# imatge-upc/rsis

Measured on AMD Instinct MI355X. Metric: training images/sec at 256x256, T=10, batch=32 per GPU, higher is better.
Workload: dtype f32

## Files before the change

include/rsis_hip.h:

```cpp
#ifndef RSIS_HIP_H
#define RSIS_HIP_H
#include <stddef.h>
#ifdef __cplusplus
extern "C" {
#endif

#define RSIS_ABI_VERSION 2

#define RSIS_DTYPE_F32 0
#define RSIS_DTYPE_BF16 1
#define RSIS_DTYPE_BF16_BLK 2
#define RSIS_DTYPE_F32_WINO 3

int rsis_version(void);
const char* rsis_error_string(int code);
int rsis_conv_uses_wino(int ks, int stride, int pad, int Cin, int Cout, int nseg, int lstm_hid);

int rsis_set_deterministic(int on);
int rsis_get_deterministic(void);

int rsis_conv_uses_bf16(int ks, int stride, int pad, int Cout);
long rsis_conv_packed_bytes_fwd(int dtype, int Cout, int ks, int stride, int pad, int nseg, const int* Cseg);
long rsis_conv_packed_bytes_dgrad(int dtype, int Cout, int ks, int stride, int pad, int c_count);
int rsis_conv_pack_fwd(const float* W, void* Wp, int Cout, int Ctot, int ks, int stride, int pad, int nseg, const int* Cseg,
// ... 52 lines not shown
typedef struct rsis_lstm_bwd_job {
  const float* dh;
  const float* dh2;
  const float* dc_next;
  const float* act;
  const float* c_prev;
  const float* c;
  float* da;
  float* dc_prev;
  int B, hid, HW;
} rsis_lstm_bwd_job;
int rsis_convlstm_bwd_gates_batch(const rsis_lstm_bwd_job* jobs, int njobs, void* stream);
typedef struct rsis_dgrad_job {
  const float* dy;
  int B, Cout, Hy, Wy;
  const void* Wd;
  int Cin_packed, ks, stride, pad;
  float* dx[3];
  int Cdx[3];
  int ndst, Hx, Wx;
  const float* addend;
  int tile, dtype;
} rsis_dgrad_job;
int rsis_conv2d_dgrad_batch(const rsis_dgrad_job* jobs, int njobs, void* stream);

int rsis_upsample_bilinear_ac_fwd(const float* x, float* y, long BC, int Hi, int Wi, int Ho, int Wo, void* stream);
int rsis_upsample_bilinear_ac_bwd(const float* dy, float* dx, long BC, int Hi, int Wi, int Ho, int Wo, void* stream);
int rsis_upsample_maxpool_bwd(const float* dy, const float* dpool, const int* argmax, float* dx, long BC, int Hi, int Wi, int Ho,
                              int Wo, void* stream);

int rsis_global_maxpool_fwd(const float* x, float* y, int* argmax, long BC, int HW, void* stream);
int rsis_global_maxpool_bwd(const float* dy, const int* argmax, float* dx, long BC, int HW, void* stream);
int rsis_global_maxpool_bwd_add(const float* dy, const int* argmax, float* dx, long BC, int HW, void* stream);

int rsis_bn_fwd(const float* x, const float* res, float* y, double* stats, const float* gamma, const float* beta,
                float* running_mean, float* running_var, float* save_mean, float* save_rstd, int B, int C, int HW,
                float eps, float momentum, int relu, int train, void* stream);
int rsis_bn_bwd(const float* dy, const float* x, const float* y, const float* save_mean, const float* save_rstd,
                const float* gamma, double* stats, float* dx, float* dres, float* dgamma, float* dbeta, int B, int C,
                int HW, int relu, void* stream);

int rsis_bn_bwd_eval(const float* dy, const float* x, const float* y, const float* running_mean, const float* running_var,
                     const float* gamma, double* stats, float* dx, float* dres, float* dgamma, float* dbeta, int B, int C, int HW,
                     float eps, int relu, void* stream);

int rsis_bn_fwd_mask(const float* x, const float* res, float* y, unsigned char* mask, double* stats, const float* gamma, const float* beta,
// ... 206 lines not shown
```

rsis_amd/_lib.py:

```python
import ctypes
import os

import torch

_HERE = os.path.dirname(os.path.abspath(__file__))
LIB_PATH = os.environ.get("RSIS_HIP_LIB") or os.path.join(_HERE, "lib", "librsis_hip.so")

_vp, _i, _l, _f = ctypes.c_void_p, ctypes.c_int, ctypes.c_long, ctypes.c_float
_ip = ctypes.POINTER(ctypes.c_int)
_vpp = ctypes.POINTER(ctypes.c_void_p)

class PackJob(ctypes.Structure):
    _fields_ = [("W", ctypes.c_void_p), ("out", ctypes.c_void_p), ("dgrad", ctypes.c_int), ("dtype", ctypes.c_int), ("Cout", ctypes.c_int),
                ("Ctot", ctypes.c_int), ("ks", ctypes.c_int), ("stride", ctypes.c_int), ("pad", ctypes.c_int),
                ("nseg", ctypes.c_int), ("Cseg", ctypes.c_int * 3), ("Coff", ctypes.c_int * 3), ("lstm_hid", ctypes.c_int),
                ("imode", ctypes.c_int), ("ldw", ctypes.c_int), ("krows", ctypes.c_int), ("block_begin", ctypes.c_int)]


class WgradJob(ctypes.Structure):
    _fields_ = [("dy", ctypes.c_void_p), ("x", ctypes.c_void_p), ("dW", ctypes.c_void_p)] + \
               [(k, ctypes.c_int) for k in ("B", "Cs", "H", "W", "Cout", "Ho", "Wo", "ks", "stride", "pad", "Ctot", "c_off", "lstm_hid", "dtype")]


class LstmJob(ctypes.Structure):
# ... 30 lines not shown


class BlkLstmBwdJob(ctypes.Structure):
    _fields_ = [(k, ctypes.c_void_p) for k in ("dh", "dh2", "dc_next", "act", "c_prev", "c", "da", "dc_prev")] + \
               [(k, ctypes.c_int) for k in ("B", "hid", "HW")]


SIGNATURES = {
    "rsis_version": (_i, []),
    "rsis_error_string": (ctypes.c_char_p, [_i]),
    "rsis_set_deterministic": (_i, [_i]),
    "rsis_get_deterministic": (_i, []),
    "rsis_conv_uses_bf16": (_i, [_i, _i, _i, _i]),
    "rsis_conv_uses_wino": (_i, [_i, _i, _i, _i, _i, _i, _i]),
    "rsis_conv_packed_bytes_fwd": (_l, [_i, _i, _i, _i, _i, _i, _ip]),
    "rsis_conv_packed_bytes_dgrad": (_l, [_i, _i, _i, _i, _i, _i]),
    "rsis_conv_pack_fwd": (_i, [_vp, _vp, _i, _i, _i, _i, _i, _i, _ip, _ip, _i, _i, _vp]),
    "rsis_conv_pack_dgrad": (_i, [_vp, _vp, _i, _i, _i, _i, _i, _i, _ip, _ip, _i, _i, _vp]),
    "rsis_conv_pack_job_fill": (_i, [ctypes.POINTER(PackJob)]),
    "rsis_conv_pack_batch": (_i, [_vp, _i, _i, _vp]),
    "rsis_conv2d_fwd": (_i, [_vpp, _ip, _i, _i, _i, _i, _vp, _i, _i, _i, _i, _vp, _vp, _vp, _i, _i, _i, _i, _vp]),
    "rsis_conv2d_fwd_bn_eval": (_i, [_vpp, _ip, _i, _i, _i, _i, _vp, _i, _i, _i, _i, _vp, _vp, _vp, _vp, _vp, _vp, _f, _i, _vp, _i, _i, _i, _i, _vp]),
    "rsis_conv2d_dgrad": (_i, [_vp, _i, _i, _i, _i, _vp, _i, _i, _i, _i, _vpp, _ip, _i, _i, _i, _vp, _i, _i, _vp]),
    "rsis_conv2d_wgrad": (_i, [_vp, _vp, _vp, _i, _i, _i, _i, _i, _i, _i, _i, _i, _i, _i, _i, _i, _i, _vp]),
    "rsis_conv2d_wgrad_batch": (_i, [ctypes.POINTER(WgradJob), _i, _vp]),
    "rsis_affine_nearest": (_i, [_vp, _vp, _vp, _i, _i, _i, _i, _i, _vp]),
    "rsis_targets_work_ints": (_l, [_i]),
    "rsis_targets_from_maps": (_i, [_vp, _vp, _i, _i, _i, _i, _vp, _vp, _vp, _vp, _vp, _vp]),
    "rsis_instance_maps_work_ints": (_l, [_i]),
    "rsis_instance_maps": (_i, [_vp, _vp, _i, _i, _i, _i, _vp, _vp, _vp, _vp]),
    "rsis_palette_to_ids": (_i, [_vp, _l, _vp, _i, _vp, _vp]),
    "rsis_idmap_rle_encode": (_i, [_vp, _i, _i, _vp, _i, _vp, _i, _vp, _vp]),
    "rsis_conv_out_wgrad": (_i, [_vp, _vp, _vp, _vp, _i, _i, _i, _i, _vp]),
    "rsis_conv_out_seq_fwd": (_i, [_vp, _vp, _vp, _vp, _i, _i, _i, _i, _i, _vp]),
    "rsis_conv_out_seq_dgrad": (_i, [_vp, _vp, _vp, _i, _i, _i, _i, _i, _vp]),
    "rsis_conv_out_seq_wgrad": (_i, [_vp, _vp, _vp, _vp, _i, _i, _i, _i, _i, _vp]),
    "rsis_sum_leading": (_i, [_vp, _vp, _i, _l, _vp]),
    "rsis_bias_grad": (_i, [_vp, _vp, _i, _i, _i, _i, _vp]),
    "rsis_convlstm_fwd": (_i, [_vpp, _ip, _i, _i, _i, _i, _vp, _vp, _vp, _vp, _vp, _vp, _vp, _i, _i, _i, _i, _i, _vp]),
    "rsis_convlstm_fwd_batch": (_i, [ctypes.POINTER(LstmJob), _i, _vp]),
    "rsis_convlstm_bwd_gates": (_i, [_vp, _vp, _vp, _vp, _vp, _vp, _vp, _vp, _vp, _i, _i, _i, _vp]),
    "rsis_upsample_bilinear_ac_fwd": (_i, [_vp, _vp, _l, _i, _i, _i, _i, _vp]),
    "rsis_upsample_bilinear_ac_bwd": (_i, [_vp, _vp, _l, _i, _i, _i, _i, _vp]),
    "rsis_upsample_maxpool_bwd": (_i, [_vp, _vp, _vp, _vp, _l, _i, _i, _i, _i, _vp]),
    "rsis_global_maxpool_fwd": (_i, [_vp, _vp, _vp, _l, _i, _vp]),
    "rsis_global_maxpool_bwd": (_i, [_vp, _vp, _vp, _l, _i, _vp]),
# ... 129 lines not shown
```

rsis_amd/csrc/api.hip:

```cpp
#include "common.h"
#include "../../include/rsis_hip.h"
#include <stdlib.h>

int rsis_launch_conv_igemm(ConvArgs& a, int ks, bool dgrad, int epi, int force_tile, hipStream_t st);
int rsis_launch_conv_wgrad(WgradArgs& a, int ks, hipStream_t st);
int rsis_launch_conv3x3_direct(ConvArgs& a, int epi, int force_variant, hipStream_t st);
int rsis_launch_conv_wino(const float* x, const void* U, const float* bias, const float* addend, float* y, int B, int C, int Cout, int H, int W,
                          hipStream_t st, int precise);
int rsis_launch_conv_wino_group(int n, const float* const* x, const void* const* U, float* const* y, float* const* y1, const int* B, const int* C,
                                const int* Cout, const int* C0, const int* H, const int* W, hipStream_t st);
int rsis_launch_convlstm_direct_group(ConvArgs* jobs, int n, const int* force_variant, hipStream_t st);
int rsis_launch_conv3x3_direct_group_plain(ConvArgs* jobs, int n, const int* force_variant, hipStream_t st);
int rsis_l_lstm_bwd_group(const void* const*, const int*, int, hipStream_t);
int rsis_launch_conv_bf16(ConvArgs& a, int ks, int epi, int force_variant, hipStream_t st);
int rsis_launch_conv_blk(ConvArgs& a, int ks, int variant, hipStream_t st);
int rsis_l_blk_from_nchw(const float*, void*, int, int, int, hipStream_t);
int rsis_l_blk_to_nchw(const void*, float*, int, int, int, hipStream_t);
long rsis_l_blk_bn_scratch(int);
int rsis_l_blk_bn_fwd(const void*, const void*, void*, double*, const float*, const float*, float*, float*, float*, float*, int, int, int, float,
                      float, int, int, hipStream_t);
int rsis_l_blk_bn_bwd(const void*, const void*, const void*, double*, const float*, const float*, const float*, const float*, void*, void*,
                      float*, float*, int, int, int, int, int, hipStream_t);
int rsis_l_blk_subsample(const void*, void*, long, int, int, int, int, int, hipStream_t);
int rsis_l_blk_upscatter(const void*, void*, long, int, int, int, int, int, hipStream_t);
// ... 394 lines not shown
  }
  if (use_direct_f2(ks, stride, pad))
    return rsis_launch_conv3x3_direct(a, 3, direct_variant(tile), (hipStream_t)stream);
  return rsis_launch_conv_igemm(a, ks, false, 0, tile, (hipStream_t)stream);
}

int rsis_conv2d_fwd(const float* const* src, const int* Csrc, int nsrc, int B, int H, int W, const void* Wp, int Cout,
                    int ks, int stride, int pad, const float* bias, const float* addend, float* out, int Ho, int Wo,
                    int tile, int dtype, void* stream) {
  return conv2d_fwd_impl(src, Csrc, nsrc, B, H, W, Wp, Cout, ks, stride, pad, bias, addend, out, Ho, Wo, tile, dtype, stream, nullptr);
}

int rsis_conv2d_fwd_bn_eval(const float* const* src, const int* Csrc, int nsrc, int B, int H, int W, const void* Wp, int Cout,
                            int ks, int stride, int pad, const float* bias, const float* addend, const float* gamma, const float* beta,
                            const float* running_mean, const float* running_var, float eps, int relu, float* out, int Ho, int Wo,
                            int tile, int dtype, void* stream) {
  const BnEval bn = {gamma, beta, running_mean, running_var, eps, relu};
  return conv2d_fwd_impl(src, Csrc, nsrc, B, H, W, Wp, Cout, ks, stride, pad, bias, addend, out, Ho, Wo, tile % 100, dtype, stream, &bn);
}

int rsis_conv2d_dgrad(const float* dy, int B, int Cout, int Hy, int Wy, const void* Wd, int Cin_packed, int ks, int stride,
                      int pad, float* const* dx, const int* Cdx, int ndst, int Hx, int Wx, const float* addend, int tile,
                      int dtype, void* stream) {
  if (!dy || !Wd || !dx || !Cdx || ndst < 1 || ndst > RSIS_MAX_SRC) return RSIS_ERR_ARG;
  const bool inplace = addend && ndst == 1 && stride > 1 && ks == 1 && pad == 0 && addend == dx[0];
  if (addend && !inplace && (ndst != 1 || stride != 1)) return RSIS_ERR_UNSUPPORTED;
  if (stride != 1 && stride != 2 && stride != 4) return RSIS_ERR_UNSUPPORTED;
  ConvArgs a = {};
  const float* srcs[1] = {dy};
  const int cs[1] = {Cout};
  int rc = fill_sources(a, srcs, cs, 1, ks);
  if (rc) return rc;
  int ctot = 0;
  for (int i = 0; i < ndst; ++i) { if (!dx[i] || Cdx[i] < 1) return RSIS_ERR_ARG; a.dst[i] = dx[i]; a.Cd[i] = Cdx[i]; ctot += Cdx[i]; }
  a.ndst = ndst;
  a.B = B; a.H = Hy; a.W = Wy; a.Ho = Hx; a.Wo = Wx; a.stride = stride; a.pad = pad; a.sshift = log2i(stride);
  if (ctot > Cin_packed) return RSIS_ERR_ARG;
  a.ostride = 1; a.oH = Hx; a.oW = Wx; a.ksplit = 1;
  a.wp = (const float*)Wd; a.ldw = rsis_roundup(Cin_packed, RSIS_LDW_ALIGN); a.Cout = ctot; a.bias = nullptr; a.addend = addend;
  if (dtype == RSIS_DTYPE_F32_WINO && wino_geom_dgrad(ks, stride, pad, Cin_packed, Cout)) {
    if (ndst > 2 || ctot % 32 != 0 || Cdx[0] % 32 != 0 || Hx != Hy || Wx != Wy || (ndst == 2 && addend)) return RSIS_ERR_UNSUPPORTED;
    if (ndst == 1) return rsis_launch_conv_wino(dy, Wd, nullptr, addend, dx[0], B, Cout, ctot, Hy, Wy, (hipStream_t)stream, 0);
    const float* xs[1] = {dy}; const void* us[1] = {Wd}; float* y0[1] = {dx[0]}; float* y1[1] = {dx[1]};
    const int b1[1] = {B}, c1[1] = {Cout}, co1[1] = {ctot}, c01[1] = {Cdx[0]}, h1[1] = {Hy}, w1[1] = {Wy};
    return rsis_launch_conv_wino_group(1, xs, us, y0, y1, b1, c1, co1, c01, h1, w1, (hipStream_t)stream);
  }
  if (use_bf16(dtype, ks, stride, pad, Cout)) {
// ... 24 lines not shown
      return rsis_l_c1_dgrad(dy, (const float*)Wd, a.ldw, dx[0], B, Cdx[0], Hx, Wx, 1, (hipStream_t)stream);
    {
      const bool splitk_ok = conv_splitk_ok();
      const int nq = (Cout + RSIS_CK - 1) / RSIS_CK;
      const long px_tiles = (long)B * rsis_cdiv(Hx, 8) * rsis_cdiv(Wx, Wx <= 8 ? 8 : 16);
      if (splitk_ok && !addend && nq >= 32 && px_tiles * rsis_cdiv(ctot, 64) < 160) {
        for (int i = 0; i < ndst; ++i)
          if (rsis_zero_async(dx[i], sizeof(float) * (size_t)B * Cdx[i] * Hx * Wx, (hipStream_t)stream) != RSIS_OK) return RSIS_ERR_LAUNCH;
        a.ksplit = 0;
      }
    }
    return rsis_launch_conv3x3_direct(a, 0, direct_variant(tile), (hipStream_t)stream);
  }
  if (use_direct_s2(ks, stride, pad) && ndst == 1 && Cdx[0] == Cin_packed && Hy == (Hx + 1) / 2 && Wy == (Wx + 1) / 2) {
    a.Ho = Hy; a.Wo = Wy; a.oH = Hx; a.oW = Wx;
    return rsis_launch_conv3x3_direct(a, 2, direct_variant(tile), (hipStream_t)stream);
  }
  if (ks == 1 && pad == 0 && stride > 1) {
    for (int i = 0; i < ndst && !inplace; ++i)
      if (rsis_zero_async(dx[i], sizeof(float) * (size_t)B * Cdx[i] * Hx * Wx, (hipStream_t)stream) != RSIS_OK) return RSIS_ERR_LAUNCH;
    a.Ho = Hy; a.Wo = Wy; a.stride = 1; a.sshift = 0; a.ostride = stride;
    return rsis_launch_conv_igemm(a, ks, false, 0, tile, (hipStream_t)stream);
  }
  return rsis_launch_conv_igemm(a, ks, true, 0, tile, (hipStream_t)stream);
}

static int wgrad_route(WgradArgs& a, int ks, int lstm_hid, int dtype) {
  if (dtype == RSIS_DTYPE_BF16_BLK) {
    a.blk = 1;
    return rsis_wgrad_bf16_supported(a, ks) ? 1 : -1;
  }
  if (use_direct(ks, a.stride, a.pad) && a.Cout == 1 && lstm_hid == 0 && rsis_c1_supported(a.Cs) && a.H == a.Ho && a.W == a.Wo && a.W % 4 == 0)
    return 0;
  if (dtype == RSIS_DTYPE_BF16 && rsis_wgrad_bf16_supported(a, ks)) return 1;
  static const bool tiled_ok = !(getenv("RSIS_WGRAD_TILED") && getenv("RSIS_WGRAD_TILED")[0] == '0');
  if (tiled_ok && rsis_wgrad_tiled_supported(a, ks)) return 2;
  return 3;
}
static int wgrad_fill(WgradArgs& a, const float* dy, const float* x, float* dW, int B, int Cs, int H, int W, int Cout, int Ho, int Wo,
                      int ks, int stride, int pad, int Ctot, int c_off, int lstm_hid) {
  if (!dy || !x || !dW || c_off < 0 || c_off + Cs > Ctot) return RSIS_ERR_ARG;
  a = WgradArgs{};
  a.dy = dy; a.x = x; a.dw = dW; a.B = B; a.Cs = Cs; a.H = H; a.W = W; a.Ho = Ho; a.Wo = Wo; a.Cout = Cout;
  a.stride = stride; a.pad = pad; a.ldo = Ctot * ks * ks; a.n_off = c_off * ks * ks; a.interleave_hid = lstm_hid;
  return RSIS_OK;
}
// ... 639 lines not shown
```

rsis_amd/csrc/common.h:

```cpp
#pragma once
#include <hip/hip_runtime.h>
#include <stdint.h>

#define RSIS_OK 0
#define RSIS_ERR_ARG 1
#define RSIS_ERR_LAUNCH 2
#define RSIS_ERR_UNSUPPORTED 3

#define RSIS_KPAD 32
#define RSIS_CK 8
#define RSIS_CKB3 16
#define RSIS_CKB1 64
#define RSIS_LDW_ALIGN 128
#define RSIS_MAX_SRC 3

typedef float f32x16 __attribute__((ext_vector_type(16)));
typedef float f32x4 __attribute__((ext_vector_type(4)));

static inline int rsis_check_launch() {
  hipError_t e = hipGetLastError();
  return e == hipSuccess ? RSIS_OK : RSIS_ERR_LAUNCH;
}

int rsis_zero_async(void* p, size_t bytes, hipStream_t st);
// ... 40 lines not shown
  int Ho, Wo;
  int stride, pad, sshift;
  const float* wp;
  int ldw;
  int Cout;
  const float* bias;
  const float* addend;
  const float* ep_gamma; const float* ep_beta; const float* ep_mean; const float* ep_var;
  float ep_eps;
  int ep_relu, ep_round;
  float* dst[RSIS_MAX_SRC];
  int Cd[RSIS_MAX_SRC];
  int ndst;
  int n_co_tiles, n_px_tiles;
  int ostride, oH, oW;
  int ksplit;
  int hid;
  const float* c_prev;
  float* h_out;
  float* c_out;
  float* act_out;
  unsigned long long* side_key;
  int precise;
};

__device__ __forceinline__ unsigned long long rsis_side_key(float v, int idx) {
  unsigned u = __float_as_uint(v);
  u = (u & 0x80000000u) ? ~u : (u | 0x80000000u);
  return ((unsigned long long)u << 32) | (unsigned)(0x7FFFFFFF - idx);
}
__device__ __forceinline__ float rsis_side_value(unsigned long long k) {
  unsigned u = (unsigned)(k >> 32);
  u = (u & 0x80000000u) ? (u & 0x7FFFFFFFu) : ~u;
  return __uint_as_float(u);
}
__device__ __forceinline__ int rsis_side_index(unsigned long long k) { return 0x7FFFFFFF - (int)(unsigned)(k & 0xFFFFFFFFull); }
__device__ __forceinline__ unsigned long long rsis_key_max32(unsigned long long k) {
#pragma unroll
  for (int o = 16; o > 0; o >>= 1) {
    const unsigned long long t = __shfl_xor(k, o, 64);
    k = t > k ? t : k;
  }
  return k;
}

#define RSIS_SIDE_CHECK_TILES 192
// ... 87 lines not shown
```

rsis_amd/csrc/conv_igemm.hip:

```cpp
#include "common.h"
#include <type_traits>

enum { EPI_PLAIN = 0, EPI_LSTM = 1, EPI_BN = 2 };
#ifndef RSIS_GEMM_NST_DEFAULT
#define RSIS_GEMM_NST_DEFAULT 2
#endif

typedef const float __attribute__((address_space(1)))* gcf_t;
typedef const char __attribute__((address_space(1)))* gcc_t;
typedef float __attribute__((address_space(1)))* gf_t;
typedef const f32x4 __attribute__((address_space(1)))* gcf4_t;

typedef __attribute__((address_space(3))) void* lds_vp_t;
template <int BM, int BN, int BK, int WGM, int WGN, int KS, bool DGRAD, int EPI, bool V4, int NST = 2>
__global__ __launch_bounds__(256) void conv_igemm_kernel(const ConvArgs p) {
#if __HIP_DEVICE_COMPILE__
  constexpr int TM = BM / WGM / 32, TN = BN / WGN / 32;
  constexpr int KK = KS * KS;
  constexpr int B_ROWS = 256 / BN;
  constexpr int B_LOADS = BK / B_ROWS;
  constexpr int A_F4 = BK * BM / 4;
  constexpr int A_LOADS = (A_F4 + 255) / 256;
  static_assert(WGM * WGN == 4, "4 waves per block");
  static_assert(BN == 64 || BN == 128 || BN == 256, "BN");
  static_assert(RSIS_KPAD % BK == 0, "BK must divide the packed K padding");
  static_assert(!V4 || (KS == 1 && !DGRAD), "V4 is the 1x1 GEMM path");
// ... 216 lines not shown
    if constexpr (V4) {
      __builtin_amdgcn_s_waitcnt(0x0F70);
    } else {
      if (more) RSIS_STORE_TILE(cur ^ 1)
    }
    __syncthreads();
  }
  }
#undef RSIS_LOAD_TILE
#undef RSIS_STORE_TILE
#undef RSIS_DMA_TILE

  if constexpr (EPI == EPI_BN) {
    if (tid < BM) {
      const int row = co_t * BM + tid;
      float sc = 0.f, sh = 0.f;
      if (row < p.Cout) rsis_bn_affine(rsis_bn_eval_rstd(p.ep_var[row], p.ep_eps), p.ep_gamma[row], p.ep_beta[row], p.ep_mean[row], sc, sh);
      lds[tid] = sc; lds[BM + tid] = sh;
    }
    __syncthreads();
  }
  const int co_base = co_t * BM + wm * TM * 32;
  const gcf_t bias = (gcf_t)p.bias, addend = (gcf_t)p.addend;
  if (EPI == EPI_PLAIN || EPI == EPI_BN) {
    const gf_t d0 = (gf_t)p.dst[0], d1 = (gf_t)p.dst[1], d2 = (gf_t)p.dst[2];
    const int Cd0 = p.Cd[0], Cd1 = p.Cd[1], Cd2 = p.Cd[2], Cout = p.Cout;
    const int e1 = Cd0, e2 = Cd0 + Cd1;
    const int ostride = p.ostride, oHW = p.oH * p.oW;
#pragma unroll
    for (int j = 0; j < TN; ++j) {
      const int opx = px_t * BN + wn * TN * 32 + j * 32 + l31;
      if (opx >= Npx) continue;
      const int ob = opx / HoWo;
      int osp = opx - ob * HoWo;
      if (ostride > 1) { const int oho = osp / Wo; osp = (oho * ostride) * p.oW + (osp - oho * Wo) * ostride; }
      if (p.ndst == 1 && (size_t)p.B * Cout * oHW * 4 < (1ull << 31)) {
        const unsigned span = (unsigned)((size_t)p.B * Cout * oHW * 4);
        const __amdgpu_buffer_rsrc_t ro = __builtin_amdgcn_make_buffer_rsrc((void*)p.dst[0], 0, span, 0x00020000);
        const __amdgpu_buffer_rsrc_t ra = __builtin_amdgcn_make_buffer_rsrc((void*)(addend ? p.addend : p.dst[0]), 0, span, 0x00020000);
        const unsigned rowb = (unsigned)oHW * 4u;
#pragma unroll
        for (int i = 0; i < TM; ++i) {
          const int row0 = co_base + i * 32 + 4 * hi;
          const unsigned vo = (unsigned)((ob * Cout + row0) * oHW + osp) * 4u;
          const int rows_left = Cout - row0;
          float av[16];
          if (addend) {
#pragma unroll
            for (int r = 0; r < 16; ++r) {
              const int k = (r & 3) + 8 * (r >> 2);
              av[r] = __builtin_bit_cast(float, __builtin_amdgcn_raw_buffer_load_b32(ra, k < rows_left ? vo + k * rowb : 0x7FFFFFF0u, 0, 0));
            }
          }
          if constexpr (EPI == EPI_BN) {
            const float* tab = lds + wm * TM * 32 + i * 32 + 4 * hi;
#pragma unroll
            for (int g = 0; g < 4; ++g) {
              const f32x4 s4 = *reinterpret_cast<const f32x4*>(tab + 8 * g), h4 = *reinterpret_cast<const f32x4*>(tab + BM + 8 * g);
#pragma unroll
              for (int kk = 0; kk < 4; ++kk) {
                const int r = 4 * g + kk, k = kk + 8 * g;
                float v = acc[i][j][r];
                if (bias) v += k < rows_left ? bias[row0 + k] : 0.f;
                v = rsis_bn_apply(v, s4[kk], h4[kk], addend ? av[r] : 0.f, p.ep_relu);
                __builtin_amdgcn_raw_buffer_store_b32(__builtin_bit_cast(unsigned, v), ro, k < rows_left ? vo + k * rowb : 0x7FFFFFF0u, 0, 0);
              }
            }
            continue;
          }
#pragma unroll
          for (int r = 0; r < 16; ++r) {
            const int k = (r & 3) + 8 * (r >> 2);
            float v = acc[i][j][r];
            if (bias) v += k < rows_left ? bias[row0 + k] : 0.f;
            if (addend) v += av[r];
            __builtin_amdgcn_raw_buffer_store_b32(__builtin_bit_cast(unsigned, v), ro, k < rows_left ? vo + k * rowb : 0x7FFFFFF0u, 0, 0);
// ... 60 lines not shown
          const size_t sidx = ((size_t)ob * hid + jh) * HoWo + osp;
          const float cp = c_prev ? c_prev[sidx] : 0.f;
          const float c = gf * cp + gi * gg;
          const float h = go * tanhf(c);
          c_out[sidx] = c;
          h_out[sidx] = h;
          if (act_out) {
            act_out[gidx] = gi; act_out[gidx + HoWo] = gf;
            act_out[gidx + 2 * (size_t)HoWo] = go; act_out[gidx + 3 * (size_t)HoWo] = gg;
          }
        }
      }
    }
  }
#endif
}

template <int BM, int BN, int BK, int WGM, int WGN, int KS, bool DGRAD, int EPI>
static int launch_cfg(ConvArgs& a, hipStream_t st) {
  const long Npx = (long)a.B * a.Ho * a.Wo;
  a.n_co_tiles = rsis_cdiv(a.Cout, BM);
  a.n_px_tiles = rsis_cdiv(Npx, BN);
  const int grid = a.n_co_tiles * 8 * rsis_cdiv(a.n_px_tiles, 8);
  if constexpr (KS == 1 && !DGRAD && (EPI == EPI_PLAIN || EPI == EPI_BN)) {
    if (a.stride == 1 && a.pad == 0 && a.nsrc == 1 && (a.H * a.W) % 4 == 0 && a.C[0] % BK == 0 &&
        (long)a.B * a.C[0] * a.H * a.W * 4 < (1L << 31)) {
      if constexpr (BM == 64 && BN == 64 && BK == 32 && EPI == EPI_PLAIN) {
        static const int nst = getenv("RSIS_GEMM_NST") ? atoi(getenv("RSIS_GEMM_NST")) : RSIS_GEMM_NST_DEFAULT;
        if (nst == 3) { hipLaunchKernelGGL((conv_igemm_kernel<BM, BN, BK, WGM, WGN, KS, DGRAD, EPI, true, 3>), dim3(grid), dim3(256), 0, st, a); return rsis_check_launch(); }
        if (nst == 4) { hipLaunchKernelGGL((conv_igemm_kernel<BM, BN, BK, WGM, WGN, KS, DGRAD, EPI, true, 4>), dim3(grid), dim3(256), 0, st, a); return rsis_check_launch(); }
      }
      hipLaunchKernelGGL((conv_igemm_kernel<BM, BN, BK, WGM, WGN, KS, DGRAD, EPI, true>), dim3(grid), dim3(256), 0, st, a);
      return rsis_check_launch();
    }
  }
  hipLaunchKernelGGL((conv_igemm_kernel<BM, BN, BK, WGM, WGN, KS, DGRAD, EPI, false>), dim3(grid), dim3(256), 0, st, a);
  return rsis_check_launch();
}

template <int KS, bool DGRAD, int EPI>
static int launch_ks(ConvArgs& a, hipStream_t st, int force_tile) {
  const long Npx = (long)a.B * a.Ho * a.Wo;
  int tile = force_tile;
  if (tile <= 0) {
    if (a.Cout <= 32) tile = (Npx >= 256L * 256) ? 1 : 2;
    else if (KS == 1) tile = 5;
    else if (a.Cout <= 64) tile = 3;
    else {
      const long b128 = (long)rsis_cdiv(a.Cout, 128) * rsis_cdiv(Npx, 128);
      tile = (b128 >= 200) ? 4 : ((b128 >= 100) ? 6 : 5);
// ... 5 lines not shown
    case 2: return launch_cfg<32, 128, 16, 1, 4, KS, DGRAD, EPI>(a, st);
    case 3: return launch_cfg<64, 128, 16, 2, 2, KS, DGRAD, EPI>(a, st);
    case 4: return launch_cfg<128, 128, 16, 2, 2, KS, DGRAD, EPI>(a, st);
    case 5: return launch_cfg<64, 64, 16, 2, 2, KS, DGRAD, EPI>(a, st);
    case 6: return launch_cfg<128, 64, 16, 2, 2, KS, DGRAD, EPI>(a, st);
    case 11: return launch_cfg<32, 256, 32, 1, 4, KS, DGRAD, EPI>(a, st);
    case 12: return launch_cfg<32, 128, 32, 1, 4, KS, DGRAD, EPI>(a, st);
    case 13: return launch_cfg<64, 128, 32, 2, 2, KS, DGRAD, EPI>(a, st);
    case 14: return launch_cfg<128, 128, 32, 2, 2, KS, DGRAD, EPI>(a, st);
    case 15: return launch_cfg<64, 64, 32, 2, 2, KS, DGRAD, EPI>(a, st);
    case 16: return launch_cfg<128, 64, 32, 2, 2, KS, DGRAD, EPI>(a, st);
    default: return RSIS_ERR_ARG;
  }
}

int rsis_launch_conv_igemm(ConvArgs& a, int ks, bool dgrad, int epi, int force_tile, hipStream_t st) {
  if (a.nsrc < 0 || a.nsrc > RSIS_MAX_SRC) return RSIS_ERR_ARG;
  if (epi == EPI_LSTM) {
    if (dgrad) return RSIS_ERR_UNSUPPORTED;
    if (ks == 3) return launch_ks<3, false, EPI_LSTM>(a, st, force_tile);
    if (ks == 1) return launch_ks<1, false, EPI_LSTM>(a, st, force_tile);
    return RSIS_ERR_UNSUPPORTED;
  }
  if (a.ep_gamma) {
    if (dgrad || epi != EPI_PLAIN || a.ndst != 1 || a.Cout <= 32 || a.Cout % 4 != 0 || (size_t)a.B * a.Cout * a.oH * a.oW * 4 >= (1ull << 31))
      return RSIS_ERR_UNSUPPORTED;
    if (ks == 1) return launch_cfg<64, 64, 32, 2, 2, 1, false, EPI_BN>(a, st);
    if (ks == 7 && a.Cout <= 64) return launch_cfg<64, 128, 32, 2, 2, 7, false, EPI_BN>(a, st);
    return RSIS_ERR_UNSUPPORTED;
  }
  if (!dgrad) {
    if (ks == 1) return launch_ks<1, false, EPI_PLAIN>(a, st, force_tile);
    if (ks == 3) return launch_ks<3, false, EPI_PLAIN>(a, st, force_tile);
    if (ks == 7) return launch_ks<7, false, EPI_PLAIN>(a, st, force_tile);
  } else {
    if (ks == 1 && a.stride == 1 && a.pad == 0) return launch_ks<1, false, EPI_PLAIN>(a, st, force_tile);
    if (ks == 1) return launch_ks<1, true, EPI_PLAIN>(a, st, force_tile);
    if (ks == 3) return launch_ks<3, true, EPI_PLAIN>(a, st, force_tile);
    if (ks == 7) return launch_ks<7, true, EPI_PLAIN>(a, st, force_tile);
  }
  return RSIS_ERR_UNSUPPORTED;
}
```

rsis_amd/ops.py:

```python
import ctypes
import os
import weakref

import torch

from . import _lib
from ._lib import check, int_array, lib, ptr, ptr_array, require_cuda_f32, stream

_WEIGHT_EPOCH = [0]


FORCE_TILE = [0]


DIRECT_GRAD = [False]


def _direct_target(param):
    g = param.grad if DIRECT_GRAD[0] and param is not None else None
    return g if (g is not None and g.is_contiguous() and g.dtype == torch.float32 and g.is_cuda) else None


DTYPE_F32, DTYPE_BF16 = 0, 1
DTYPE_F32_WINO = 3
# ... 161 lines not shown
            L = lib()
            Cout, Ctot = w.shape[0], w.shape[1]
            nseg, segs, offs = self._seg_args()
            n = L.rsis_conv_packed_bytes_dgrad(self.dtype, Cout, self.ks, self.stride, self.pad, self.cin) // 4
            if self.wd is None or self.wd.numel() != n:
                self.wd = torch.zeros(n, dtype=torch.float32, device=w.device)
            check(L.rsis_conv_pack_dgrad(ptr(w.detach()), ptr(self.wd), Cout, Ctot, self.ks, self.stride, self.pad, nseg, segs, offs,
                                         self.lstm_hid, self.dtype, stream()), "rsis_conv_pack_dgrad")
            self._key_d = key
            if self._refs is None:
                self._refs = (weakref.ref(w), None)
            _PACKS.add(self)
        return self.wd


def _contig(t):
    return t if t.is_contiguous() else t.contiguous()


def _conv_out_size(n, ks, stride, pad):
    return (n + 2 * pad - ks) // stride + 1


def _dgrad_all(L, dy, wd, cin_packed, ks, stride, pad, srcs, Hx, Wx, addend=None, inplace=False, dtype=DTYPE_F32):
    B, Cout, Hy, Wy = dy.shape
    shapes = [tuple(s.shape) if torch.is_tensor(s) else tuple(s) for s in srcs]
    dxs = [addend] if inplace else [torch.empty(sh, dtype=torch.float32, device=dy.device) for sh in shapes]
    check(L.rsis_conv2d_dgrad(ptr(dy), B, Cout, Hy, Wy, ptr(wd), cin_packed, ks, stride, pad, ptr_array(dxs),
                              int_array([sh[1] for sh in shapes]), len(shapes), Hx, Wx, ptr(addend), FORCE_TILE[0], dtype, stream()),
          "rsis_conv2d_dgrad")
    return dxs


class GradSlot(object):

    def __init__(self):
        self.grad = None
        self.done = False

    def reset(self):
        self.grad, self.done = None, False

    def take(self):
        g, self.grad = self.grad, None
        self.done = True
        return g

    def park(self, g):
        if self.done or self.grad is not None or g is None:
            return False
        self.grad = g
        return True


class _GradTapFn(torch.autograd.Function):
    @staticmethod
    def forward(ctx, x, slot):
        ctx.slot = slot
        return x.view_as(x)

    @staticmethod
    def backward(ctx, g):
        if g is not None and ctx.slot.park(g if g.is_contiguous() else g.contiguous()):
            return None, None
        return g, None


def grad_tap(x, slot):
    if slot is None or not (torch.is_grad_enabled() and x.requires_grad):
        return x
    return _GradTapFn.apply(x, slot)


WGRAD_DEFER = [False]
_WGRAD_QUEUE = []
# ... 23 lines not shown
def _wgrad_all(L, dy, srcs, w_shape, ks, stride, pad, lstm_hid, out=None, dtype=DTYPE_F32):
    B, Cout, Ho, Wo = dy.shape
    Ctot = w_shape[1]
    dW = out if out is not None else torch.zeros(w_shape, dtype=torch.float32, device=dy.device)
    c_off = 0
    for s in srcs:
        _, Cs, H, W = s.shape
        wgrad_launch(L, dy, s, dW, B, Cs, H, W, Cout, Ho, Wo, ks, stride, pad, Ctot, c_off, lstm_hid, dtype, "rsis_conv2d_wgrad",
                     out is not None)
        c_off += Cs
    return dW


class _Conv2dFn(torch.autograd.Function):
    @staticmethod
    def forward(ctx, pack, stride, pad, nsrc, slot, *tensors):
        srcs = [_contig(t) for t in tensors[:nsrc]]
        weight, bias = tensors[nsrc], tensors[nsrc + 1]
        ctx.slot = slot
        require_cuda_f32(weight, bias, *srcs)
        L = lib()
        B, _, H, W = srcs[0].shape
        Cout, ks = weight.shape[0], weight.shape[2]
        Ho, Wo = _conv_out_size(H, ks, stride, pad), _conv_out_size(W, ks, stride, pad)
        if pack.stride != stride or pack.pad != pad:
            raise _lib.RsisHipError("PackedConv was built for stride %d pad %d, used with %d/%d" % (pack.stride, pack.pad, stride, pad))
        wp = pack.fwd(weight)
        out = torch.empty((B, Cout, Ho, Wo), dtype=torch.float32, device=weight.device)
        ctx.in_shape = None
        if ks == 1 and stride > 1 and pad == 0 and nsrc == 1 and (SUBSAMPLE_1X1[0] or pack.dtype == DTYPE_BF16):
            ctx.in_shape = tuple(srcs[0].shape)
            sub = torch.empty((B, srcs[0].shape[1], Ho, Wo), dtype=torch.float32, device=weight.device)
            check(L.rsis_subsample2d(ptr(srcs[0]), ptr(sub), B * srcs[0].shape[1], H, W, stride, stream()), "rsis_subsample2d")
            srcs = [sub]
            H, W, stride_k = Ho, Wo, 1
        else:
            stride_k = stride
        tile = FORCE_TILE[0] + (100 if pack.training_call else 0)
        check(L.rsis_conv2d_fwd(ptr_array(srcs), int_array([s.shape[1] for s in srcs]), nsrc, B, H, W, ptr(wp), Cout, ks, stride_k,
                                pad, ptr(bias.detach() if bias is not None else None), None, ptr(out), Ho, Wo, tile, pack.dtype, stream()),
              "rsis_conv2d_fwd")
        ctx.pack, ctx.stride, ctx.pad, ctx.nsrc = pack, stride, pad, nsrc
        ctx.has_bias = bias is not None
        ctx.wparam, ctx.bparam = weight, bias
        ctx.save_for_backward(weight, *srcs)
        return out

    @staticmethod
    def backward(ctx, dy):
        weight = ctx.saved_tensors[0]
        srcs = list(ctx.saved_tensors[1:])
        dy = _contig(dy)
        L = lib()
        ks = weight.shape[2]
        nsrc = ctx.nsrc
        grads = [None] * (nsrc + 2)
        take, park = ctx.slot if isinstance(ctx.slot, tuple) else (ctx.slot, None)
        addend = take.take() if take is not None else None
        sub = ctx.in_shape is not None
        in_shapes = [ctx.in_shape] if sub else [tuple(t.shape) for t in srcs]
        if any(ctx.needs_input_grad[5:5 + nsrc]):
            wd = ctx.pack.dgrad(weight)
            inplace, extra = False, None
            if addend is not None:
                if nsrc != 1 or tuple(addend.shape) != in_shapes[0]:
                    raise _lib.RsisHipError("GradSlot: the parked gradient does not belong to this conv's input")
                if ctx.stride != 1:
                    if ks == 1 and ctx.pad == 0 and addend.is_contiguous():
                        inplace = True
                    else:
                        extra, addend = addend, None
            dxs = _dgrad_all(L, dy, wd, ctx.pack.cin, ks, ctx.stride, ctx.pad, in_shapes, in_shapes[0][2], in_shapes[0][3], addend,
                             inplace, dtype=ctx.pack.dtype)
            if extra is not None:
                dxs[0].add_(extra)
            for i in range(nsrc):
                if ctx.needs_input_grad[5 + i]:
                    grads[i] = dxs[i]
            if park is not None and nsrc == 1 and grads[0] is not None and park.park(grads[0]):
                grads[0] = None
        want_w = ctx.needs_input_grad[5 + nsrc]
        want_b = ctx.has_bias and ctx.needs_input_grad[6 + nsrc]
        if (want_w and want_b and weight.shape[0] == 1 and ks == 3 and ctx.stride == 1 and ctx.pad == 1 and nsrc == 1 and
                weight.shape[1] in (4, 8, 16) and srcs[0].shape[3] % 4 == 0):
            tw, tb = _direct_target(ctx.wparam), _direct_target(ctx.bparam)
            dW = tw if tw is not None else torch.zeros_like(weight)
            db = tb if tb is not None else torch.zeros(1, dtype=torch.float32, device=dy.device)
            x0 = srcs[0]
            check(L.rsis_conv_out_wgrad(ptr(dy), ptr(x0), ptr(dW), ptr(db), x0.shape[0], x0.shape[1], x0.shape[2], x0.shape[3], stream()),
                  "rsis_conv_out_wgrad")
            grads[nsrc] = None if tw is not None else dW
            grads[nsrc + 1] = None if tb is not None else db
            return (None, None, None, None, None) + tuple(grads)
        if want_w:
            tgt = _direct_target(ctx.wparam)
            dW = _wgrad_all(L, dy, srcs, tuple(weight.shape), ks, 1 if sub else ctx.stride, ctx.pad, 0, out=tgt, dtype=ctx.pack.dtype)
# ... 225 lines not shown
        x, y, gamma, mean, rstd = ctx.saved_tensors
        dy = _contig(dy)
        B, C, H, W = x.shape
        if not ctx.train:
            stats = torch.empty(2 * C, dtype=torch.float64, device=dy.device)
            dx = torch.empty_like(x)
            need_dres = ctx.has_res and ctx.relu
            dres = torch.empty_like(x) if need_dres else None
            dgamma = torch.empty(C, dtype=torch.float32, device=dy.device)
            dbeta = torch.empty_like(dgamma)
            fn, name = (lib().rsis_bn_bwd_eval_mask, "rsis_bn_bwd_eval_mask") if ctx.masked else (lib().rsis_bn_bwd_eval, "rsis_bn_bwd_eval")
            check(fn(ptr(dy), ptr(x), ptr(y), ptr(mean), ptr(rstd), ptr(gamma.detach()), ptr(stats), ptr(dx), ptr(dres),
                     ptr(dgamma), ptr(dbeta), B, C, H * W, float(ctx.eps), int(ctx.relu), stream()), name)
            if ctx.has_res and not need_dres:
                dres = dy
            return dx, dres, dgamma, dbeta, None, None, None, None, None, None, None, None, None
        flags = int(ctx.relu)
        if ctx.arena is not None:
            stats, flags = ctx.arena[1], flags | 2
        else:
            stats = torch.empty(2 * C, dtype=torch.float64, device=dy.device)
        dx = torch.empty_like(x)
        need_dres = ctx.has_res and ctx.relu
        dres = torch.empty_like(x) if need_dres else None
        tg, tb = _direct_target(ctx.gparam), _direct_target(ctx.bparam)
        direct = tg is not None and tb is not None
        if direct:
            dgamma, dbeta, flags = tg, tb, flags | 4
        else:
            dgamma = torch.empty(C, dtype=torch.float32, device=dy.device)
            dbeta = torch.empty_like(dgamma)
        fn, name = (lib().rsis_bn_bwd_mask, "rsis_bn_bwd_mask") if ctx.masked else (lib().rsis_bn_bwd, "rsis_bn_bwd")
        check(fn(ptr(dy), ptr(x), ptr(y), ptr(mean), ptr(rstd), ptr(gamma.detach()), ptr(stats), ptr(dx), ptr(dres),
                 ptr(dgamma), ptr(dbeta), B, C, H * W, flags, stream()), name)
        if ctx.has_res and not need_dres:
            dres = dy
        if direct:
            dgamma = dbeta = None
        if ctx.res_slot is not None and ctx.res_slot.park(dres):
            dres = None
        return dx, dres, dgamma, dbeta, None, None, None, None, None, None, None, None, None


def batchnorm(x, gamma, beta, running_mean, running_var, train, relu=False, res=None, eps=1e-5, momentum=0.1, arena=None,
              res_slot=None):
    want_grad = torch.is_grad_enabled() and any(t is not None and t.requires_grad for t in (x, res, gamma, beta))
    return _BatchNormFn.apply(x, res, gamma, beta, running_mean, running_var, bool(train), bool(relu), eps, momentum, arena,
                              res_slot if (train and res is not None) else None, want_grad)


class _MaxPool3x3s2Fn(torch.autograd.Function):
    @staticmethod
    def forward(ctx, x, slot=None):
        ctx.slot = slot
        x = _contig(x)
        require_cuda_f32(x)
        B, C, H, W = x.shape
        Ho, Wo = _conv_out_size(H, 3, 2, 1), _conv_out_size(W, 3, 2, 1)
        y = torch.empty((B, C, Ho, Wo), dtype=torch.float32, device=x.device)
        arg = torch.empty((B, C, Ho, Wo), dtype=torch.uint8, device=x.device)
        check(lib().rsis_maxpool3x3s2_fwd(ptr(x), ptr(y), ptr(arg), B * C, H, W, Ho, Wo, stream()), "rsis_maxpool3x3s2_fwd")
        ctx.save_for_backward(arg)
# ... 389 lines not shown
```

Before: 961.5.

## Fuse masked residual gradient into 1x1 conv dgrad epilogue

Adds a masked-addend epilogue to the 1x1 implicit-GEMM dgrad kernel. Instead of the BN backward writing a full dres tensor (dy masked by ReLU), the BN backward parks dy plus a byte mask, and the downstream conv dgrad applies the mask while adding. This removes one full activation-sized write and read plus an allocation per residual block, at the cost of extra byte-mask loads in the epilogue and a more complex slot handoff protocol.

```diff
diff --git a/include/rsis_hip.h b/include/rsis_hip.h
--- a/include/rsis_hip.h
+++ b/include/rsis_hip.h
@@ -98,6 +98,9 @@
   const float* addend;
   int tile, dtype;
 } rsis_dgrad_job;
+int rsis_conv2d_dgrad_masked(const float* dy, int B, int Cout, int Hy, int Wy, const void* Wd, int Cin_packed, int ks, int stride,
+                             int pad, float* const* dx, const int* Cdx, int ndst, int Hx, int Wx, const float* addend,
+                             const unsigned char* addend_mask, int tile, int dtype, void* stream);
 int rsis_conv2d_dgrad_batch(const rsis_dgrad_job* jobs, int njobs, void* stream);
 
 int rsis_upsample_bilinear_ac_fwd(const float* x, float* y, long BC, int Hi, int Wi, int Ho, int Wo, void* stream);
diff --git a/rsis_amd/_lib.py b/rsis_amd/_lib.py
--- a/rsis_amd/_lib.py
+++ b/rsis_amd/_lib.py
@@ -76,6 +76,7 @@
     "rsis_conv2d_fwd": (_i, [_vpp, _ip, _i, _i, _i, _i, _vp, _i, _i, _i, _i, _vp, _vp, _vp, _i, _i, _i, _i, _vp]),
     "rsis_conv2d_fwd_bn_eval": (_i, [_vpp, _ip, _i, _i, _i, _i, _vp, _i, _i, _i, _i, _vp, _vp, _vp, _vp, _vp, _vp, _f, _i, _vp, _i, _i, _i, _i, _vp]),
     "rsis_conv2d_dgrad": (_i, [_vp, _i, _i, _i, _i, _vp, _i, _i, _i, _i, _vpp, _ip, _i, _i, _i, _vp, _i, _i, _vp]),
+    "rsis_conv2d_dgrad_masked": (_i, [_vp, _i, _i, _i, _i, _vp, _i, _i, _i, _i, _vpp, _ip, _i, _i, _i, _vp, _vp, _i, _i, _vp]),
     "rsis_conv2d_wgrad": (_i, [_vp, _vp, _vp, _i, _i, _i, _i, _i, _i, _i, _i, _i, _i, _i, _i, _i, _i, _vp]),
     "rsis_conv2d_wgrad_batch": (_i, [ctypes.POINTER(WgradJob), _i, _vp]),
     "rsis_affine_nearest": (_i, [_vp, _vp, _vp, _i, _i, _i, _i, _i, _vp]),
diff --git a/rsis_amd/csrc/api.hip b/rsis_amd/csrc/api.hip
--- a/rsis_amd/csrc/api.hip
+++ b/rsis_amd/csrc/api.hip
@@ -440,7 +440,15 @@
 int rsis_conv2d_dgrad(const float* dy, int B, int Cout, int Hy, int Wy, const void* Wd, int Cin_packed, int ks, int stride,
                       int pad, float* const* dx, const int* Cdx, int ndst, int Hx, int Wx, const float* addend, int tile,
                       int dtype, void* stream) {
-  if (!dy || !Wd || !dx || !Cdx || ndst < 1 || ndst > RSIS_MAX_SRC) return RSIS_ERR_ARG;
+  return rsis_conv2d_dgrad_masked(dy, B, Cout, Hy, Wy, Wd, Cin_packed, ks, stride, pad, dx, Cdx, ndst, Hx, Wx, addend, nullptr, tile, dtype, stream);
+}
+int rsis_conv2d_dgrad_masked(const float* dy, int B, int Cout, int Hy, int Wy, const void* Wd, int Cin_packed, int ks, int stride,
+                             int pad, float* const* dx, const int* Cdx, int ndst, int Hx, int Wx, const float* addend,
+                             const unsigned char* addend_mask, int tile, int dtype, void* stream) {
+  if (!dy || !Wd || !dx || !Cdx || ndst < 1 || ndst > RSIS_MAX_SRC || (addend_mask && !addend)) return RSIS_ERR_ARG;
+  if (addend_mask && (dtype != RSIS_DTYPE_F32 || ks != 1 || stride != 1 || pad != 0 || ndst != 1 || Hx != Hy || Wx != Wy || (Hx * Wx) % 4 != 0 ||
+                      Cdx[0] < 1 || (size_t)B * Cdx[0] * Hx * Wx * 4 >= (1ull << 31)))
+    return RSIS_ERR_UNSUPPORTED;
   const bool inplace = addend && ndst == 1 && stride > 1 && ks == 1 && pad == 0 && addend == dx[0];
   if (addend && !inplace && (ndst != 1 || stride != 1)) return RSIS_ERR_UNSUPPORTED;
   if (stride != 1 && stride != 2 && stride != 4) return RSIS_ERR_UNSUPPORTED;
@@ -511,6 +519,7 @@
     a.Ho = Hy; a.Wo = Wy; a.stride = 1; a.sshift = 0; a.ostride = stride;
     return rsis_launch_conv_igemm(a, ks, false, 0, tile, (hipStream_t)stream);
   }
+  if (addend_mask) { a.addend_mask = addend_mask; return rsis_launch_conv_igemm(a, ks, true, 3 , tile, (hipStream_t)stream); }
   return rsis_launch_conv_igemm(a, ks, true, 0, tile, (hipStream_t)stream);
 }
 
diff --git a/rsis_amd/csrc/common.h b/rsis_amd/csrc/common.h
--- a/rsis_amd/csrc/common.h
+++ b/rsis_amd/csrc/common.h
@@ -86,6 +86,7 @@
   float* act_out;
   unsigned long long* side_key;
   int precise;
+  const unsigned char* addend_mask;
 };
 
 __device__ __forceinline__ unsigned long long rsis_side_key(float v, int idx) {
diff --git a/rsis_amd/csrc/conv_igemm.hip b/rsis_amd/csrc/conv_igemm.hip
--- a/rsis_amd/csrc/conv_igemm.hip
+++ b/rsis_amd/csrc/conv_igemm.hip
@@ -1,7 +1,7 @@
 #include "common.h"
 #include <type_traits>
 
-enum { EPI_PLAIN = 0, EPI_LSTM = 1, EPI_BN = 2 };
+enum { EPI_PLAIN = 0, EPI_LSTM = 1, EPI_BN = 2, EPI_MASKADD = 3 };
 #ifndef RSIS_GEMM_NST_DEFAULT
 #define RSIS_GEMM_NST_DEFAULT 2
 #endif
@@ -264,7 +264,7 @@
   }
   const int co_base = co_t * BM + wm * TM * 32;
   const gcf_t bias = (gcf_t)p.bias, addend = (gcf_t)p.addend;
-  if (EPI == EPI_PLAIN || EPI == EPI_BN) {
+  if (EPI == EPI_PLAIN || EPI == EPI_BN || EPI == EPI_MASKADD) {
     const gf_t d0 = (gf_t)p.dst[0], d1 = (gf_t)p.dst[1], d2 = (gf_t)p.dst[2];
     const int Cd0 = p.Cd[0], Cd1 = p.Cd[1], Cd2 = p.Cd[2], Cout = p.Cout;
     const int e1 = Cd0, e2 = Cd0 + Cd1;
@@ -294,6 +294,23 @@
               av[r] = __builtin_bit_cast(float, __builtin_amdgcn_raw_buffer_load_b32(ra, k < rows_left ? vo + k * rowb : 0x7FFFFFF0u, 0, 0));
             }
           }
+          if constexpr (EPI == EPI_MASKADD) {
+            const __amdgpu_buffer_rsrc_t rm = __builtin_amdgcn_make_buffer_rsrc((void*)p.addend_mask, 0, span >> 4, 0x00020000);
+            unsigned mk[16];
+#pragma unroll
+            for (int r = 0; r < 16; ++r) {
+              const int k = (r & 3) + 8 * (r >> 2);
+              mk[r] = __builtin_amdgcn_raw_buffer_load_b8(rm, k < rows_left ? (vo + k * rowb) >> 4 : 0x7FFFFFF0u, 0, 0);
+            }
+#pragma unroll
+            for (int r = 0; r < 16; ++r) {
+              const int k = (r & 3) + 8 * (r >> 2);
+              const unsigned o = vo + k * rowb;
+              const float v = acc[i][j][r] + (((mk[r] >> ((o >> 2) & 3u)) & 1u) ? av[r] : 0.f);
+              __builtin_amdgcn_raw_buffer_store_b32(__builtin_bit_cast(unsigned, v), ro, k < rows_left ? o : 0x7FFFFFF0u, 0, 0);
+            }
+            continue;
+          }
           if constexpr (EPI == EPI_BN) {
             const float* tab = lds + wm * TM * 32 + i * 32 + 4 * hi;
 #pragma unroll
@@ -400,10 +417,10 @@
   a.n_co_tiles = rsis_cdiv(a.Cout, BM);
   a.n_px_tiles = rsis_cdiv(Npx, BN);
   const int grid = a.n_co_tiles * 8 * rsis_cdiv(a.n_px_tiles, 8);
-  if constexpr (KS == 1 && !DGRAD && (EPI == EPI_PLAIN || EPI == EPI_BN)) {
+  if constexpr (KS == 1 && !DGRAD && (EPI == EPI_PLAIN || EPI == EPI_BN || EPI == EPI_MASKADD)) {
     if (a.stride == 1 && a.pad == 0 && a.nsrc == 1 && (a.H * a.W) % 4 == 0 && a.C[0] % BK == 0 &&
         (long)a.B * a.C[0] * a.H * a.W * 4 < (1L << 31)) {
-      if constexpr (BM == 64 && BN == 64 && BK == 32 && EPI == EPI_PLAIN) {
+      if constexpr (BM == 64 && BN == 64 && BK == 32 && (EPI == EPI_PLAIN || EPI == EPI_MASKADD)) {
         static const int nst = getenv("RSIS_GEMM_NST") ? atoi(getenv("RSIS_GEMM_NST")) : RSIS_GEMM_NST_DEFAULT;
         if (nst == 3) { hipLaunchKernelGGL((conv_igemm_kernel<BM, BN, BK, WGM, WGN, KS, DGRAD, EPI, true, 3>), dim3(grid), dim3(256), 0, st, a); return rsis_check_launch(); }
         if (nst == 4) { hipLaunchKernelGGL((conv_igemm_kernel<BM, BN, BK, WGM, WGN, KS, DGRAD, EPI, true, 4>), dim3(grid), dim3(256), 0, st, a); return rsis_check_launch(); }
@@ -455,6 +472,12 @@
     if (ks == 1) return launch_ks<1, false, EPI_LSTM>(a, st, force_tile);
     return RSIS_ERR_UNSUPPORTED;
   }
+  if (epi == EPI_MASKADD) {
+    if (ks != 1 || a.stride != 1 || a.pad != 0 || a.ndst != 1 || !a.addend || !a.addend_mask || a.bias || a.ostride != 1 || (a.oH * a.oW) % 4 != 0 ||
+        (size_t)a.B * a.Cout * a.oH * a.oW * 4 >= (1ull << 31))
+      return RSIS_ERR_UNSUPPORTED;
+    return launch_ks<1, false, EPI_MASKADD>(a, st, force_tile);
+  }
   if (a.ep_gamma) {
     if (dgrad || epi != EPI_PLAIN || a.ndst != 1 || a.Cout <= 32 || a.Cout % 4 != 0 || (size_t)a.B * a.Cout * a.oH * a.oW * 4 >= (1ull << 31))
       return RSIS_ERR_UNSUPPORTED;
diff --git a/rsis_amd/ops.py b/rsis_amd/ops.py
--- a/rsis_amd/ops.py
+++ b/rsis_amd/ops.py
@@ -207,10 +207,15 @@
     return (n + 2 * pad - ks) // stride + 1
 
 
-def _dgrad_all(L, dy, wd, cin_packed, ks, stride, pad, srcs, Hx, Wx, addend=None, inplace=False, dtype=DTYPE_F32):
+def _dgrad_all(L, dy, wd, cin_packed, ks, stride, pad, srcs, Hx, Wx, addend=None, inplace=False, dtype=DTYPE_F32, addend_mask=None):
     B, Cout, Hy, Wy = dy.shape
     shapes = [tuple(s.shape) if torch.is_tensor(s) else tuple(s) for s in srcs]
     dxs = [addend] if inplace else [torch.empty(sh, dtype=torch.float32, device=dy.device) for sh in shapes]
+    if addend_mask is not None:
+        check(L.rsis_conv2d_dgrad_masked(ptr(dy), B, Cout, Hy, Wy, ptr(wd), cin_packed, ks, stride, pad, ptr_array(dxs),
+                                         int_array([sh[1] for sh in shapes]), len(shapes), Hx, Wx, ptr(addend), ptr(addend_mask), FORCE_TILE[0], dtype,
+                                         stream()), "rsis_conv2d_dgrad_masked")
+        return dxs
     check(L.rsis_conv2d_dgrad(ptr(dy), B, Cout, Hy, Wy, ptr(wd), cin_packed, ks, stride, pad, ptr_array(dxs),
                               int_array([sh[1] for sh in shapes]), len(shapes), Hx, Wx, ptr(addend), FORCE_TILE[0], dtype, stream()),
           "rsis_conv2d_dgrad")
@@ -221,21 +226,33 @@
 
     def __init__(self):
         self.grad = None
+        self.mask = None
         self.done = False
+        self.masked_ok = False
 
     def reset(self):
-        self.grad, self.done = None, False
-
-    def take(self):
-        g, self.grad = self.grad, None
+        self.grad, self.mask, self.done, self.masked_ok = None, None, False, False
+
+    def take(self, with_mask=False):
+        g, m, self.grad, self.mask = self.grad, self.mask, None, None
         self.done = True
+        if with_mask:
+            return g, m
+        if m is not None:
+            raise _lib.RsisHipError("GradSlot: a masked gradient was parked for a consumer that cannot take one")
         return g
 
-    def park(self, g):
-        if self.done or self.grad is not None or g is None:
+    def can_park(self):
+        return not (self.done or self.grad is not None)
+
+    def park(self, g, mask=None):
+        if not self.can_park() or g is None:
             return False
-        self.grad = g
+        self.grad, self.mask = g, mask
         return True
+
+
+BN_DRES = [os.environ.get("RSIS_BN_DRES", "0") == "1"]
 
 
 class _GradTapFn(torch.autograd.Function):
@@ -305,6 +322,10 @@
         L = lib()
         B, _, H, W = srcs[0].shape
         Cout, ks = weight.shape[0], weight.shape[2]
+        take = slot[0] if isinstance(slot, tuple) else slot
+        if take is not None:
+            take.masked_ok = (pack.dtype == DTYPE_F32 and ks == 1 and stride == 1 and pad == 0 and nsrc == 1 and (H * W) % 4 == 0 and
+                              srcs[0].numel() * 4 < (1 << 31) and not BN_DRES[0])
         Ho, Wo = _conv_out_size(H, ks, stride, pad), _conv_out_size(W, ks, stride, pad)
         if pack.stride != stride or pack.pad != pad:
             raise _lib.RsisHipError("PackedConv was built for stride %d pad %d, used with %d/%d" % (pack.stride, pack.pad, stride, pad))
@@ -339,7 +360,7 @@
         nsrc = ctx.nsrc
         grads = [None] * (nsrc + 2)
         take, park = ctx.slot if isinstance(ctx.slot, tuple) else (ctx.slot, None)
-        addend = take.take() if take is not None else None
+        addend, amask = take.take(with_mask=True) if take is not None else (None, None)
         sub = ctx.in_shape is not None
         in_shapes = [ctx.in_shape] if sub else [tuple(t.shape) for t in srcs]
         if any(ctx.needs_input_grad[5:5 + nsrc]):
@@ -354,7 +375,7 @@
                     else:
                         extra, addend = addend, None
             dxs = _dgrad_all(L, dy, wd, ctx.pack.cin, ks, ctx.stride, ctx.pad, in_shapes, in_shapes[0][2], in_shapes[0][3], addend,
-                             inplace, dtype=ctx.pack.dtype)
+                             inplace, dtype=ctx.pack.dtype, addend_mask=amask)
             if extra is not None:
                 dxs[0].add_(extra)
             for i in range(nsrc):
@@ -626,7 +647,9 @@
             stats = torch.empty(2 * C, dtype=torch.float64, device=dy.device)
         dx = torch.empty_like(x)
         need_dres = ctx.has_res and ctx.relu
-        dres = torch.empty_like(x) if need_dres else None
+        slot = ctx.res_slot
+        lazy = need_dres and ctx.masked and slot is not None and slot.masked_ok and slot.can_park() and not BN_DRES[0]
+        dres = torch.empty_like(x) if need_dres and not lazy else None
         tg, tb = _direct_target(ctx.gparam), _direct_target(ctx.bparam)
         direct = tg is not None and tb is not None
         if direct:
@@ -641,7 +664,10 @@
             dres = dy
         if direct:
             dgamma = dbeta = None
-        if ctx.res_slot is not None and ctx.res_slot.park(dres):
+        if lazy:
+            if not slot.park(dy, y):
+                raise _lib.RsisHipError("GradSlot: the masked hand-over was refused after it had been granted")
+        elif ctx.res_slot is not None and ctx.res_slot.park(dres):
             dres = None
         return dx, dres, dgamma, dbeta, None, None, None, None, None, None, None, None, None
 
```

Result: no change. 965.5 (median of 6 runs) (+0.4%).
